# haowenz/chromap

Measured on AMD Instinct MI355X. Metric: M paired reads mapped/s (ATAC preset, GRCh38 index), higher is better.
Workload: dtype u64

## Files before the change

chromap_amd/csrc/cm_api.hip:

```cpp
#include <hip/hip_runtime.h>
#include <math.h>
#include <stdio.h>
#include <stdlib.h>
#include <string.h>

#include <string>
#include <vector>

#include "../../include/chromap_amd.h"
#include "cm_barcode_translate.h"
#include "cm_ctx.h"
#include "cm_kernels.h"
#include "cm_classes.h"
#include "cm_summary.h"
#include "cm_coop.h"
#include <chrono>
#include <mutex>
#include "cm_mapq_tables.h"

static thread_local std::string g_last_error;

static bool cm_debug_pool() { static const bool on = getenv("CM_DEBUG_POOL") != nullptr; return on; }
static thread_local std::string t_last_error;
void cm_set_error(cmgpu_ctx *ctx, const std::string &msg) {
// ... 90 lines not shown
    c->opt.spec = value ? 1 : 0;
    if (value < 0) { c->cls_seen = 0; memset(c->cls_age, 0, sizeof(c->cls_age)); }
  } else if (n == "debug_candidate_capacity") {
    if (value > 0 && cm_ensure_candidate_arrays(c, (uint64_t)value)) { cm_set_error(c, "out of device memory (candidates)"); return CMGPU_ENOMEM; }
    c->pred_m_ok = value > 0; c->m_cap = (uint64_t)value; c->pred_n = 0xffffffffu;
  } else if (n == "coop_profile") {
    if (value) { if (c->coop_prof.ensure(64 * 8)) return CMGPU_ENOMEM; CM_HIPCHECK(c, hipMemset(c->coop_prof.p, 0, 64 * 8)); } else c->coop_prof.release();
  } else if (n == "coop_run_table") {
    c->opt.coop_rb = (int)value;
  } else if (n == "coop") {
    c->opt.coop = (int)value;
  } else if (n == "pack_once") {
    c->opt.pack_once = value ? 1 : 0;
  } else if (n == "s3b_short") {
    c->opt.s3b_short = value ? 1 : 0;
  } else if (n == "s6_planes") {
    c->opt.s6_planes = value ? 1 : 0;
  } else if (n == "generic_kernels") {
    c->opt.generic_kernels = value ? 1 : 0;
  } else if (n == "item_limit") {
    c->opt.item_limit = value > 0 ? (uint64_t)value : 0xfffffff0ull;
  } else {
    cm_set_error(c, "unknown option " + n);
    return CMGPU_EINVAL;
  }
  return CMGPU_OK;
}

extern "C" int cmgpu_get_option(const cmgpu_ctx *c, const char *name, int64_t *value) {
  if (!c || !name || !value) return CMGPU_EINVAL;
  const std::string n(name);
  if (n == "probe_lookups_per_lane") *value = c->opt.probe_variant & 15;
  else if (n == "probe_pair_prefetch") *value = (c->opt.probe_variant & 16) ? 1 : 0;
  else if (n == "mm_chunks") *value = c->opt.mm_chunks;
  else if (n == "h2d_copy_blocks") *value = c->opt.h2d_kernel;
  else if (n == "d2h_copy_blocks") *value = c->opt.d2h_kernel;
  else if (n == "prep_kernel") *value = c->opt.prep_kernel;
  else if (n == "prep_tile_reads") *value = c->opt.prep_tile_reads;
  else if (n == "item_limit") *value = (int64_t)c->opt.item_limit;
  else if (n == "lanes") *value = c->opt.lanes;
  else if (n == "coop") *value = c->opt.coop;
  else if (n == "generic_kernels") *value = c->opt.generic_kernels;
  else if (n == "s3b_short") *value = c->opt.s3b_short;
  else if (n == "pack_once") *value = c->opt.pack_once;
  else if (n == "s6_planes") *value = c->opt.s6_planes;
  else if (n == "alloc_us") *value = (int64_t)(c->alloc_seconds * 1e6);
  else if (n == "alloc_draw_us") *value = (int64_t)(c->alloc_draw_seconds * 1e6);
  else if (n.rfind("coop_profile_", 0) == 0) {
    const int k = atoi(n.c_str() + 13);
    unsigned long long v = 0;
    if (k < 0 || k > 63 || !c->coop_prof.p || hipMemcpy(&v, (const unsigned long long *)c->coop_prof.p + k, 8, hipMemcpyDeviceToHost) != hipSuccess) return CMGPU_EINVAL;
    *value = (int64_t)v;
  }
  else if (n == "probe_table_buckets") *value = c->fmask ? (int64_t)c->fmask + 1 : (int64_t)c->bmask + 1;
  else return CMGPU_EINVAL;
  return CMGPU_OK;
}

extern "C" const char *cmgpu_last_error(const cmgpu_ctx *ctx) { return ctx ? ctx->err.c_str() : g_last_error.c_str(); }
// ... 658 lines not shown
  }
  return CMGPU_OK;
}
struct MmChunks {
  uint32_t n_chunks;
  uint32_t lo[CM_MM_CHUNKS + 1];
  uint64_t entries[CM_MM_CHUNKS];
  uint32_t part_off[CM_MM_CHUNKS + 1];
};
static uint32_t mm_chunk_count(const RangeRun &r) { return r.n >= (1u << 20) ? (uint32_t)r.c->opt.mm_chunks : (r.n >= (1u << 17) ? 2 : 1); }
static void mm_probe_grids(const cmgpu_ctx *c, MmChunks &k) {
  k.part_off[0] = 0;
  for (uint32_t ch = 0; ch < k.n_chunks; ++ch) k.part_off[ch + 1] = k.part_off[ch] + cm_probe_range_blocks(k.entries[ch], c->opt.probe_variant);
}
template <class Fill>
static int mm_fill_and_probe(RangeRun &r, const MmChunks &k, uint32_t mm_cap, Fill fill) {
  cmgpu_ctx *c = r.c;
  const unsigned long long *marks = (const unsigned long long *)c->mm_marks.p;
  CM_HIPCHECK(c, hipMemsetAsync(r.d.stats + CM_ST_PROBE_STEPS, 0, 2 * 8, r.s));
  for (uint32_t ch = 0; ch < k.n_chunks; ++ch) {
    fill(ch);
    CM_HIPCHECK(c, hipEventRecord(c->chunk_ev[ch], r.s));
    CM_HIPCHECK(c, hipStreamWaitEvent(c->stream2, c->chunk_ev[ch], 0));
    cm_launch_k_probe_range(r.d, marks + ch, k.entries[ch], mm_cap, (uint2 *)c->partials.p + k.part_off[ch], c->stream2, c->opt.probe_variant);
  }
  CM_HIPCHECK(c, hipEventRecord(c->chunk_ev[CM_MM_CHUNKS], c->stream2));
  CM_HIPCHECK(c, hipStreamWaitEvent(r.s, c->chunk_ev[CM_MM_CHUNKS], 0));
  cm_launch_k_probe_reduce(c->partials.p, k.part_off[k.n_chunks], r.d.stats + CM_ST_PROBE_STEPS, r.s);
  return CMGPU_OK;
}
static bool range_wants_planes(const cmgpu_ctx *c) { return c->ref_pl_words != 0 && c->opt.planes; }
static size_t read_planes_bytes(const cmgpu_ctx *c, uint32_t n2) { return (size_t)n2 * cm_read_pl_stride((c->max_read_len + 31) / 32) * 4 + 16; }
static int stage_minimizers_fused(RangeRun &r, bool flat) {
  cmgpu_ctx *c = r.c; CmDev &d = r.d; hipStream_t s = r.s;
  const uint32_t n = r.n, n2 = r.n2;
  int rc;
  const bool pl = !flat && c->opt.pack_once && cm_prep_mm_planes_supported(d, c->max_read_len);
  if (pl && range_wants_planes(c) && !c->read_planes.ensure(read_planes_bytes(c, n2))) {
    d.read_pl = (uint32_t *)c->read_planes.p; d.read_pl_w = (c->max_read_len + 31) / 32;
// ... 18 lines not shown
      chunk_pairs = pairs > chunk_pairs ? pairs : chunk_pairs;
      const uint64_t me = 2ull * pairs * (attempt == 0 ? (uint64_t)(c->max_read_len / 4 + 3) : per_read_bound);
      k.entries[ch] = me > cap ? cap : me;
    }
    mm_probe_grids(c, k);
    if (c->mm_hash.ensure((size_t)cap * 8 + 8) || c->mm_ps.ensure((size_t)cap * 4 + 4) || c->pr_val.ensure((size_t)cap * 8 + 8) ||
        (!flat && c->mm_stage.ensure(cm_prep_mm_stage_bytes(d, c->max_read_len, chunk_pairs) + 8)) ||
        c->pr_kind.ensure((size_t)cap + 4) || c->mm_cursor.ensure(8) || c->mm_marks.ensure((CM_MM_CHUNKS + 1) * 8) ||
        c->partials.ensure(((size_t)k.part_off[k.n_chunks] + 1) * 8 + cm_stats_partial_words(n) * 8)) {
      cm_set_error(c, "out of device memory (minimizers)"); return CMGPU_ENOMEM;
    }
    r.bind();
    CM_HIPCHECK(c, hipMemsetAsync(c->mm_cursor.p, 0, 8, s));
    CM_HIPCHECK(c, hipMemsetAsync(c->mm_marks.p, 0, 8, s));
    unsigned long long *cursor = (unsigned long long *)c->mm_cursor.p, *marks = (unsigned long long *)c->mm_marks.p;
    rc = mm_fill_and_probe(r, k, (uint32_t)cap, [&](uint32_t ch) {
      if (flat) cm_launch_k_prep_flat(d, k.lo[ch], k.lo[ch + 1], c->max_read_len, (uint32_t)c->opt.prep_tile_reads, (uint32_t)cap, cursor, s);
      else cm_launch_k_prep_mm(d, k.lo[ch], k.lo[ch + 1], c->max_read_len, (uint32_t)cap, cursor, s, c->mm_stage.p, pl);
      cm_launch_k_copy_u64(cursor, marks + ch + 1, s);
    });
    if (rc) return rc;
    d.mm_cap = (uint32_t)cap;
    CM_HIPCHECK(c, hipMemsetAsync(c->hv_cnt.p, 0, 256, s));
    cm_launch_k_s3a_count(d, n2, s);
    d.mm_cap = 0;
    if ((rc = scan_with_total(c, d.hit_tot, d.hit_off, n2, &r.hits_total, false))) return rc;
    CM_HIPCHECK(c, hipMemcpyAsync(r.n_heavy, c->hv_cnt.p, sizeof(r.n_heavy), hipMemcpyDeviceToHost, s));
    r.s3a_done = true;
    unsigned long long hm[CM_MM_CHUNKS + 1];
    CM_HIPCHECK(c, hipMemcpyAsync(hm, marks, ((size_t)k.n_chunks + 1) * 8, hipMemcpyDeviceToHost, s));
    CM_HIPCHECK(c, cm_stream_sync(s));
    const unsigned long long tot = hm[k.n_chunks];
    bool grid_short = false;
    if (attempt == 0 && tot <= cap)
      for (uint32_t ch = 0; ch < k.n_chunks; ++ch) grid_short = grid_short || hm[ch + 1] - hm[ch] > k.entries[ch];
    if (tot <= cap && !grid_short) { r.n_mm = (uint32_t)tot; break; }
    if (attempt == 1) { cm_set_error(c, "minimizer arrays overflowed twice"); return CMGPU_ECAPACITY; }
    cap = bound;
  }
  mark(c, "s0_s1_s2_trim_minimizers_probe");
// ... 38 lines not shown
    (void)hipDeviceGetStreamPriorityRange(&prio_least, &prio_greatest);
    CM_HIPCHECK(c, hipStreamCreateWithPriority(&c->stream_pack, hipStreamNonBlocking, prio_greatest));
  }
  CM_HIPCHECK(c, hipEventRecord(c->chunk_ev[1], r.s));
  CM_HIPCHECK(c, hipStreamWaitEvent(c->stream_pack, c->chunk_ev[1], 0));
  r.d.read_pl = (uint32_t *)c->read_planes.p; r.d.read_pl_w = (c->max_read_len + 31) / 32;
  cm_launch_k_pack_reads(r.d, r.n2, c->stream_pack);
  CM_HIPCHECK(c, hipEventRecord(c->chunk_ev[0], c->stream_pack));
  return CMGPU_OK;
}
static int stage_s3_candidates(RangeRun &r) {
  cmgpu_ctx *c = r.c; CmDev &d = r.d; hipStream_t s = r.s;
  const uint32_t n2 = r.n2;
  if (!r.s3a_done) {
    CM_HIPCHECK(c, hipMemsetAsync(c->hv_cnt.p, 0, 256, s));
    cm_launch_k_s3a_count(d, n2, s);
    CM_HIPCHECK(c, hipMemcpyAsync(r.n_heavy, c->hv_cnt.p, sizeof(r.n_heavy), hipMemcpyDeviceToHost, s));
    const int rc = scan_with_total(c, d.hit_tot, d.hit_off, n2, &r.hits_total);
    if (rc) return rc;
  }
  if (r.hits_total > r.limit) return CM_RC_SPLIT;
  r.n_hits = (uint32_t)r.hits_total;
  if (c->hbuf.ensure((size_t)r.n_hits * 8 + 8) || c->hcnt.ensure((size_t)r.n_hits + 4)) { cm_set_error(c, "out of device memory (hits)"); return CMGPU_ENOMEM; }
  r.bind();
  mark(c, "s3a_count");
  cm_launch_k_s3b_candidates(d, n2, c->max_read_len, s);
  const uint32_t *nh = r.n_heavy;
  cm_launch_k_s3b_heavy(d, nh, s, (c->opt.coop & 1) != 0, c->max_read_len);
  c->use_perm = (uint64_t)nh[CM_L_HIT_B256B] + nh[CM_L_HIT_SLAB] + nh[CM_L_HIT_B512] + nh[CM_L_HIT_B1024] > n2 / 65536 || (uint64_t)nh[CM_L_HIT_WAVE] + nh[CM_L_HIT_WAVE_SMALL] + nh[CM_L_HIT_B256A] > n2 / 256;
  if (c->opt.heavy_last) c->use_perm = c->opt.heavy_last > 0;
  if (c->use_perm) {
// ... 472 lines not shown
    if (c->last_range_lo != 0 || c->last_range_hi != c->n_pairs) { cm_set_error(c, "the batch was mapped in sub-batches"); return CMGPU_EINVAL; }
    if (capacity < n || !c->read_planes.p || c->read_planes.cap < n * 4) { cm_set_error(c, "debug array: buffer too small or array not resident"); return CMGPU_ECAPACITY; }
    CM_HIPCHECK(c, hipMemcpy(out, c->read_planes.p, n * 4, hipMemcpyDeviceToHost));
    return CMGPU_OK;
  }
  if (nm == "read_plain") {
    const uint64_t n = 2ull * c->n_pairs;
    if (n_out) *n_out = n;
    if (c->last_range_lo != 0 || c->last_range_hi != c->n_pairs) { cm_set_error(c, "the batch was mapped in sub-batches"); return CMGPU_EINVAL; }
    if (capacity < n || !c->read_plain.p || c->read_plain.cap < n) { cm_set_error(c, "debug array: buffer too small or array not resident"); return CMGPU_ECAPACITY; }
    std::vector<uint8_t> b(n);
    if (n) CM_HIPCHECK(c, hipMemcpy(b.data(), c->read_plain.p, n, hipMemcpyDeviceToHost));
    for (uint64_t i = 0; i < n; ++i) out[i] = b[i];
    return CMGPU_OK;
  }
  struct { const char *n; DevBuf *b; int per_pair; } tab[] = {
    {"rlen", &c->rlen, 0}, {"mm_cnt", &c->mm_cnt, 0}, {"hit_tot", &c->hit_tot, 0}, {"ncp", &c->ncp, 0}, {"ncn", &c->ncn, 0},
    {"resc_p", &c->resc_p, 0}, {"resc_n", &c->resc_n, 0}, {"mcp", &c->mcp, 0}, {"mcn", &c->mcn, 0}, {"fcp", &c->fcp, 0},
    {"fcn", &c->fcn, 0}, {"ndp", &c->ndp, 0}, {"ndn", &c->ndn, 0}, {"nv", &c->nv, 0}, {"pe_nbest", &c->pe_nbest, 1}};
  for (auto &t : tab)
    if (nm == t.n) {
      const uint64_t n = t.per_pair ? c->n_pairs : 2ull * c->n_pairs;
      if (n_out) *n_out = n;
      if (capacity < n || !t.b->p || t.b->cap < n * 4) { cm_set_error(c, "debug array: buffer too small or array not resident"); return CMGPU_ECAPACITY; }
      CM_HIPCHECK(c, hipMemcpy(out, t.b->p, n * 4, hipMemcpyDeviceToHost));
      return CMGPU_OK;
    }
  cm_set_error(c, "debug array: unknown name " + nm);
  return CMGPU_EINVAL;
}

extern "C" int cmgpu_debug_mapq(cmgpu_ctx *c, int kind, int32_t error_threshold, uint64_t n, const int32_t *reads, const int32_t *pairs,
// ... 603 lines not shown
```

chromap_amd/csrc/cm_ctx.h:

```cpp
#ifndef CM_CTX_H_
#define CM_CTX_H_
#include <hip/hip_runtime.h>

#include <string>
#include <thread>
#include <vector>

#include "../../include/chromap_amd.h"
#include "../../include/chromap_amd_debug.h"
#include "cm_types.h"

#define CM_MAX_EVENTS 32
#define CM_MAX_W_HOST 32
#define CM_BZ_SRC_NONE 0
#define CM_BZ_SRC_STORE 1
#define CM_BZ_SRC_UPLOAD 2
#define CM_BZ_SRC_DEVICE 3

struct DevBuf {
  void *p = nullptr;
  size_t cap = 0;
  bool owned = true;
  int ensure(size_t bytes);
  void release();
// ... 92 lines not shown
  int probe_variant = 1;
  int mm_chunks = CM_MM_CHUNKS;
  int prep_tile_reads = 32;
  int prep_kernel = 0;
  uint64_t item_limit = 0xfffffff0ull;
  int exchange_overlap = 0;
  int s3b_cap = 0;
  int lanes = 1;
  int heavy_mid = 0;
  int heavy_max[3] = {0, 0, 0};
  int heavy_last = 0;
  int spec = 1;
  int pack_once = 1;
  int s6_planes = 1;
  int s3b_short = 1;
  int generic_kernels = 0;
  int coop_rb = 0;
  int coop = 0xff;
};

struct cmgpu_ctx {
  CmOptions opt;
  int device = 0;
  hipStream_t stream = nullptr;
  hipStream_t stream2 = nullptr;
  hipStream_t stream_pack = nullptr;
  hipEvent_t chunk_ev[CM_MM_CHUNKS + 1] = {};
  std::string err;
  cmgpu_params hp;
  CmParams p;
// ... 191 lines not shown
```

chromap_amd/csrc/cm_kernels.h:

```cpp
#ifndef CM_KERNELS_H_
#define CM_KERNELS_H_
#include <hip/hip_runtime.h>

#include "cm_types.h"

#define CM_SLAB_CAP 65535u
#define CM_SLAB_BLOCKS 128u
#define CM_DECL_LAUNCH(kname) void cm_launch_##kname(const CmDev &d, uint32_t n, hipStream_t s);
void cm_launch_k_prep_count(const CmDev &d, uint32_t n_pairs, uint32_t max_read_len, hipStream_t s);
void cm_launch_k_mm_fill(const CmDev &d, uint32_t pair_lo, uint32_t pair_hi, uint32_t max_read_len, hipStream_t s);
void cm_launch_k_mm_marks(const uint32_t *mm_off, const uint32_t *lo, uint32_t n_marks, unsigned long long *marks, hipStream_t s);
bool cm_prep_mm_supported(const CmDev &d, uint32_t max_read_len);
bool cm_prep_flat_supported(const CmDev &d, uint32_t max_read_len, uint32_t tile_reads);
void cm_launch_k_prep_flat(const CmDev &d, uint32_t pair_lo, uint32_t pair_hi, uint32_t max_read_len, uint32_t tile_reads, uint32_t mm_cap,
                           unsigned long long *cursor, hipStream_t s);
uint32_t cm_prep_mm_pairs_per_block(const CmDev &d, uint32_t max_read_len);
size_t cm_prep_mm_stage_bytes(const CmDev &d, uint32_t max_read_len, uint32_t pairs);
bool cm_prep_mm_planes_supported(const CmDev &d, uint32_t max_read_len);
void cm_launch_k_prep_mm(const CmDev &d, uint32_t pair_lo, uint32_t pair_hi, uint32_t max_read_len, uint32_t mm_cap,
                         unsigned long long *cursor, hipStream_t s, void *gstage, bool planes = false);
uint32_t cm_probe_range_blocks(uint64_t max_entries, int variant);
void cm_launch_k_probe_range(const CmDev &d, const unsigned long long *range, uint64_t max_entries, uint32_t cap, void *partials, hipStream_t s, int variant);
void cm_launch_k_probe_reduce(const void *partials, uint32_t blocks, unsigned long long *counters, hipStream_t s);
CM_DECL_LAUNCH(k_s3a_count)
void cm_launch_k_sort_lists(const CmDev &d, int mode, hipStream_t s);
uint32_t cm_s3b_lane_cap(uint32_t max_read_len);
void cm_s3b_heavy_classes(uint32_t *hv_max, uint32_t *hv_big);
void cm_granted_classes(CmDev &d);
void cm_launch_k_s3b_heavy(const CmDev &d, const uint32_t *n_cls, hipStream_t s, bool coop, uint32_t max_read_len);
void cm_launch_k_s3b_candidates(const CmDev &d, uint32_t n, uint32_t max_read_len, hipStream_t s);
void cm_launch_k_s4a_rescue_count(const CmDev &d, uint32_t n, hipStream_t s, bool coop);
void cm_launch_k_s4b_rescue_merge(const CmDev &d, uint32_t n, hipStream_t s, bool coop, uint32_t max_read_len);
uint32_t cm_rescue_seg_cap(uint32_t n_reads);
void cm_launch_k_s4a_rescue_list(const CmDev &d, uint32_t n_reads, hipStream_t s, bool coop);
void cm_launch_k_s4b_rescue_list(const CmDev &d, uint32_t n_reads, hipStream_t s, bool coop, uint32_t max_read_len);
void cm_launch_k_s4c_reduce(const CmDev &d, uint32_t n, hipStream_t s, uint32_t coop);
void cm_launch_k_s5a_prepare(const CmDev &d, uint32_t n, hipStream_t s, bool coop);
void cm_launch_k_s5c_finalize(const CmDev &d, uint32_t n, hipStream_t s, bool coop);
void cm_launch_k_s5b_verify(const CmDev &d, uint32_t max_items, uint32_t n_reads, hipStream_t s);
// ... 29 lines not shown
```

chromap_amd/csrc/cm_kernels.hip:

```cpp
#include <hip/hip_runtime.h>
#include <stdio.h>
#include <string.h>
#include <cstring>
#include <atomic>
#include <map>
#include <mutex>
#include <type_traits>
#include <utility>
#include <rocprim/rocprim.hpp>

#include "cm_kernels.h"
#include "cm_stages.h"
#include "cm_classes.h"
#include "cm_coop.h"

#define CM_BLOCK 256

#define CM_ITEM_KERNEL(kname, fn, perm)                                      \
  __global__ __launch_bounds__(CM_BLOCK) void kname(CmDev d, uint32_t n) {   \
    if (d.abort && *d.abort) return;                                         \
    const uint32_t i = blockIdx.x * CM_BLOCK + threadIdx.x;                  \
    if (i < n) fn(d, d.perm ? d.perm[i] : i);                                \
  }

// ... 307 lines not shown
      d.mm_cnt[r] = (uint32_t)pref[b] - (uint32_t)pref[a];
      d.mm_off[r] = (uint32_t)(base + pref[a]);
    }
    __syncthreads();
  }
  if (valid && ri[t].fb) {
    const uint8_t *seq = cm_read_ptr(d, r);
    const uint32_t c = cm_minimizers_window<7>(seq, len, k, nullptr, nullptr, 0);
    const unsigned long long off = c ? atomicAdd(cursor, (unsigned long long)c) : 0ull;
    d.mm_cnt[r] = c;
    d.mm_off[r] = (uint32_t)off;
    if (c && off + c <= mm_cap) cm_minimizers_window<7>(seq, len, k, d.mm_hash + off, d.mm_ps + off, c);
  }
}

__global__ __launch_bounds__(CM_BLOCK) void k_s3a_count(CmDev d, uint32_t n) {
  const uint32_t i = blockIdx.x * CM_BLOCK + threadIdx.x;
  uint32_t tot = 0;
  if (i < n) {
    cm_s3a_count(d, i);
    tot = d.hit_tot[i];
  }
  const uint32_t cls = cm_hit_class(d, tot);
  __shared__ uint32_t sh_cnt[8], sh_base[8];
  if (threadIdx.x < 8) sh_cnt[threadIdx.x] = 0;
  __syncthreads();
  const uint32_t lane = threadIdx.x & 63u;
  const uint32_t ids[8] = {CM_L_HIT_WAVE, CM_L_HIT_B256A, CM_L_HIT_B256B, CM_L_HIT_SLAB, CM_L_HIT_G16, CM_L_HIT_B512, CM_L_HIT_WAVE_SMALL, CM_L_HIT_B1024};
  uint32_t slot = 0, mine = 8;
#pragma unroll
  for (uint32_t q = 0; q < 8; ++q) {
    const unsigned long long m = __ballot(cls == ids[q]);
// ... 1217 lines not shown
  }
}
void cm_launch_k_sum_u32(const uint32_t *in, uint32_t n, unsigned long long *out, hipStream_t s) {
  if (!n) return;
  uint32_t blocks = (n + CM_BLOCK * 8 - 1) / (CM_BLOCK * 8);
  if (blocks > 2048) blocks = 2048;
  hipLaunchKernelGGL(k_sum_u32, dim3(blocks), dim3(CM_BLOCK), 0, s, in, n, out);
}

static inline dim3 grid_for(uint32_t n) { return dim3((n + CM_BLOCK - 1) / CM_BLOCK); }

#define CM_LAUNCH(kname)                                                               \
  void cm_launch_##kname(const CmDev &d, uint32_t n, hipStream_t s) {                  \
    if (n) hipLaunchKernelGGL(kname, grid_for(n), dim3(CM_BLOCK), 0, s, d, n);         \
  }
void cm_launch_k_s3a_count(const CmDev &d, uint32_t n, hipStream_t s) {
  if (n) hipLaunchKernelGGL(k_s3a_count, grid_for(n), dim3(CM_BLOCK), 0, s, d, n);
}
uint32_t cm_s3b_lane_cap(uint32_t max_read_len) {
  uint32_t cap = max_read_len / 3;
  return cap < 16 ? 16 : (cap > 64 ? 64 : cap);
}
static inline bool cm_cls_on(const CmDev &d, uint32_t list) { return (d.cls_mask >> list) & 1ull; }
template <class K>
static bool cm_lds_optin(K kernel, size_t bytes) {
  if (bytes <= 64 * 1024) return true;
  if (bytes > 160 * 1024) return false;
  static std::mutex mu;
  static std::map<std::pair<int, const void *>, std::pair<size_t, size_t>> seen;
  int dev = 0;
  (void)hipGetDevice(&dev);
  std::lock_guard<std::mutex> lk(mu);
// ... 437 lines not shown
```

chromap_amd/csrc/cm_stages.h:

```cpp
#ifndef CM_STAGES_H_
#define CM_STAGES_H_

#include "cm_types.h"

struct CmModeAny {
  static constexpr bool kPe = false;
  static CM_HD bool split(const CmDev &d) { return d.p.split != 0; }
  static CM_HD bool single(const CmDev &d) { return d.p.single != 0; }
};
struct CmModePe {
  static constexpr bool kPe = true;
  static CM_HD bool split(const CmDev &) { return false; }
  static CM_HD bool single(const CmDev &) { return false; }
};

CM_HD uint32_t cm_c2u(uint8_t c) {
  const uint32_t u = c & 0xDFu;
  const uint32_t x = (u >> 1) & 3u;
  const uint32_t o = u - 0x41u;
  const bool acgt = o < 20u && ((0x80045u >> (o & 31u)) & 1u);
  return acgt ? x ^ (x >> 1) : 4u;
}
CM_HD uint8_t cm_negchar(uint8_t c) {
  const uint32_t v = 3u ^ cm_c2u(c);
// ... 411 lines not shown
  *s0_out = fa ? sa : sb;
  return true;
}

CM_HD uint32_t cm_brev32(uint32_t v);
CM_HD uint64_t cm_brev64(uint64_t v) { return ((uint64_t)cm_brev32((uint32_t)v) << 32) | cm_brev32((uint32_t)(v >> 32)); }
CM_HD uint64_t cm_mask64(uint32_t n) { return n >= 64u ? ~0ull : ((1ull << n) - 1ull); }
CM_HD void cm_trim_planes64(uint64_t a0, uint64_t a1, uint32_t l1, uint64_t b0, uint64_t b1, uint32_t l2, int min_overlap, int seed,
                            bool *found, uint32_t *s0_out) {
  const uint32_t down = 64u - l2;
  uint64_t B0 = ~(cm_brev64(b0) >> down), B1 = ~(cm_brev64(b1) >> down);
  const uint64_t seedmask = cm_mask64((uint32_t)seed);
  bool fa = false, fb = false;
  uint32_t sa = 0, sb = 0;
  const uint32_t last = l2 - (uint32_t)min_overlap;
  for (uint32_t s0 = 0; s0 <= last && !fa; ++s0) {
    const uint32_t n = l1 < l2 - s0 ? l1 : l2 - s0;
    const uint64_t D = ((a0 ^ B0) | (a1 ^ B1)) & cm_mask64(n);
    const bool ok = __builtin_popcountll(D) <= 1;
    if (ok && (D & seedmask) == 0) { fa = true; sa = s0; }
    if (ok && ((D >> seed) & seedmask) == 0 && !fb) { fb = true; sb = s0; }
    B0 >>= 1; B1 >>= 1;
  }
  *found = fa || fb;
  *s0_out = fa ? sa : sb;
}
struct CmPairPlanes { uint64_t p0[2], p1[2]; bool upper[2]; };

CM_HD void cm_s0_prep_ptr(const CmDev &d, uint32_t pair, const uint8_t *s1p, const uint8_t *s2p, const CmPairPlanes *pp = nullptr) {
  const uint32_t raw1 = d.ro0[pair + 1] - d.ro0[pair], raw2 = d.ro1[pair + 1] - d.ro1[pair];
  uint32_t len1 = raw1, len2 = raw2;
  bool ok = raw1 >= (uint32_t)d.p.min_read_len && (d.p.single || raw2 >= (uint32_t)d.p.min_read_len);
  if (d.bcb && !d.bc_ok[pair] && !d.p.bc_keep) ok = false;
  if (ok && d.p.trim && !d.p.single) {
    const uint8_t *s1 = s1p, *s2 = s2p;
    const bool swap = !(raw1 <= raw2);
    const uint8_t *rd1 = swap ? s2 : s1;
    const uint8_t *lng = swap ? s1 : s2;
    const uint32_t l1 = swap ? raw2 : raw1, l2 = swap ? raw1 : raw2;
    const int min_overlap = d.p.min_read_len;
    const int seed = min_overlap / 2;
    bool merged = false;
    bool fast = false, ffound = false;
    uint32_t fs0 = 0;
    if (seed >= 1 && seed <= 32 && 2 * seed <= min_overlap && l1 >= (uint32_t)min_overlap) {
      if (pp && l2 <= 64) {
        const int ia = swap ? 1 : 0, ib = swap ? 0 : 1;
        fast = pp->upper[0] && pp->upper[1];
        if (fast) cm_trim_planes64(pp->p0[ia], pp->p1[ia], l1, pp->p0[ib], pp->p1[ib], l2, min_overlap, seed, &ffound, &fs0);
      } else if (l2 <= 64) fast = cm_trim_fast<2>(rd1, l1, lng, l2, min_overlap, seed, &ffound, &fs0);
      else if (l2 <= 160) fast = cm_trim_fast<5>(rd1, l1, lng, l2, min_overlap, seed, &ffound, &fs0);
      else if (l2 <= 256) fast = cm_trim_fast<8>(rd1, l1, lng, l2, min_overlap, seed, &ffound, &fs0);
    }
    if (fast) {
      merged = true;
      if (ffound) {
        int overlap = (int)(l2 - fs0);
        int off2 = 0;
        if (overlap > (int)l1) { off2 = overlap - (int)l1; overlap = (int)l1; }
        const int t1 = swap ? overlap + off2 : overlap;
// ... 115 lines not shown
    if (ctl(pos, c < 4 ? 2 : 0)) { flush = false; break; }
  }
  if (flush && min_h != ~0ull) CM_EMIT(min_h, min_p);
#undef CM_EMIT
  return n;
}

template <int W, class Emit>
CM_HD uint32_t cm_minimizers_window_e(const uint8_t *seq, uint32_t len, int k, Emit &&emit) {
  return cm_minimizers_core<W>(seq, 0, len, true, k, W, [&](uint32_t n, uint64_t h, uint32_t p) { emit(n, h, p); return true; });
}

struct CmSrcBytes {
  const uint8_t *seq;
  CM_HD uint32_t operator()(uint32_t i) const { return cm_c2u(seq[i]); }
};
struct CmSrcPlanes {
  uint64_t p0, p1;
  CM_HD uint32_t operator()(uint32_t i) const { return ((uint32_t)(p0 >> i) & 1u) | (((uint32_t)(p1 >> i) & 1u) << 1); }
};
template <class Src, class Emit>
CM_HD uint32_t cm_minimizers_w7_oddk_seq_src(const Src &src, uint32_t len, int k, Emit &&emit) {
  const uint64_t shift = 2 * (uint64_t)(k - 1);
  const uint64_t mask = (((uint64_t)1) << (2 * k)) - 1;
  uint64_t fw = 0, rv = 0;
  uint64_t H[7];
#pragma unroll
  for (int j = 0; j < 7; ++j) H[j] = ~0ull;
  uint32_t sb = 0, fl = 0, bad = 0, n = 0;
  for (uint32_t pos = 0; pos < len; ++pos) {
    uint32_t c = src(pos);
    bad |= c >> 2;
    c &= 3;
    fw = ((fw << 2) | c) & mask;
// ... 32 lines not shown
  if (m_k < 7) {
    uint64_t v = ~0ull;
    int at = -1;
#pragma unroll
    for (int j = 0; j < 7; ++j)
      if (j >= 7 - (int)m_k && H[j] <= v) { v = H[j]; at = j; }
    if (at >= 0) { emit(n, v, ((len - 1 - (uint32_t)(6 - at)) << 1) | ((sb >> at) & 1u)); ++n; }
    return n;
  }
#pragma unroll
  for (int j = 0; j < 7; ++j)
    if ((fl >> j) & 1u) { emit(n, H[j], ((len - 1 - (uint32_t)(6 - j)) << 1) | ((sb >> j) & 1u)); ++n; }
  return n;
}

template <int HV, class Src, class Emit>
CM_HD uint32_t cm_minimizers_w7_oddk_blocks_src(const Src &src, uint32_t len, int k, Emit &&emit) {
  const uint64_t shift = 2 * (uint64_t)(k - 1);
  const uint64_t mask = (((uint64_t)1) << (2 * k)) - 1;
  uint64_t fw = 0, rv = 0;
  uint32_t bad = 0, n = 0;
  for (uint32_t pos = 0; pos + 1 < (uint32_t)k; ++pos) {
    uint32_t c = src(pos);
    bad |= c >> 2;
    c &= 3;
    fw = ((fw << 2) | c) & mask;
    rv = (rv >> 2) | (((uint64_t)(3 ^ c)) << shift);
  }
  const uint32_t m = len - (uint32_t)k + 1, nblk = (m + 6) / 7;
  uint64_t ep[7], Sp[7], SM[7];
  uint32_t sbp = 0;
#pragma unroll
  for (int j = 0; j < 7; ++j) { ep[j] = 0; Sp[j] = 0; SM[j] = 0; }
  for (uint32_t b = 0; b <= nblk; ++b) {
    uint64_t e[7];
    uint32_t sb = 0;
#pragma unroll
    for (int j = 0; j < 7; ++j) {
      const uint32_t i = 7 * b + (uint32_t)j;
      e[j] = 0;
      if (i < m) {
        uint32_t c = src(i + (uint32_t)k - 1);
        bad |= c >> 2;
        c &= 3;
        fw = ((fw << 2) | c) & mask;
        rv = (rv >> 2) | (((uint64_t)(3 ^ c)) << shift);
        const uint64_t h0 = cm_hash64_v<HV>(fw, mask), h1 = cm_hash64_v<HV>(rv, mask);
        const uint32_t strand = h0 < h1 ? 0u : 1u;
        e[j] = cm_hash64_v<HV>(strand ? h1 : h0, mask);
        sb |= strand << j;
      }
    }
    if (b == 0) {
      uint64_t v = e[0];
#pragma unroll
      for (int j = 1; j < 6; ++j) v = e[j] < v ? e[j] : v;
      if (e[6] == v) {
#pragma unroll
        for (int j = 0; j < 6; ++j) e[j] = e[j] == v ? ~0ull : e[j];
      }
    }
    uint64_t Mw[7];
    {
      uint64_t P = e[0];
      Mw[0] = Sp[0];
#pragma unroll
      for (int j = 1; j < 7; ++j) {
        Mw[j] = Sp[j] < P ? Sp[j] : P;
        P = e[j] < P ? e[j] : P;
      }
    }
    if (b > 0) {
      uint64_t PM = Mw[0];
#pragma unroll
      for (int j = 0; j < 7; ++j) {
        if (j > 0) PM = Mw[j] > PM ? Mw[j] : PM;
        const uint64_t F = j < 6 ? (SM[j < 6 ? j + 1 : 6] > PM ? SM[j < 6 ? j + 1 : 6] : PM) : PM;
        const uint32_t i = 7 * (b - 1) + (uint32_t)j;
        if (F == ep[j] && i < m) { emit(n, ep[j], ((i + (uint32_t)k - 1) << 1) | ((sbp >> j) & 1u)); ++n; }
      }
    }
    SM[6] = Mw[6];
    Sp[6] = e[6];
#pragma unroll
    for (int j = 5; j >= 0; --j) {
      SM[j] = Mw[j] > SM[j + 1] ? Mw[j] : SM[j + 1];
      Sp[j] = e[j] < Sp[j + 1] ? e[j] : Sp[j + 1];
    }
#pragma unroll
    for (int j = 0; j < 7; ++j) ep[j] = e[j];
    sbp = sb;
  }
  if (bad) return ~0u;
  return n;
}
template <class Src, class Emit>
CM_HD uint32_t cm_minimizers_w7_oddk_src(const Src &src, uint32_t len, int k, Emit &&emit) {
  if (len < (uint32_t)k + 6) return cm_minimizers_w7_oddk_seq_src(src, len, k, emit);
  if (2 * k == 34) return cm_minimizers_w7_oddk_blocks_src<0>(src, len, k, emit);
  if (2 * k > 32 && 2 * k <= 52) return cm_minimizers_w7_oddk_blocks_src<1>(src, len, k, emit);
  return cm_minimizers_w7_oddk_blocks_src<2>(src, len, k, emit);
}
template <class Emit>
CM_HD uint32_t cm_minimizers_w7_oddk_seq(const uint8_t *seq, uint32_t len, int k, Emit &&emit) {
  return cm_minimizers_w7_oddk_seq_src(CmSrcBytes{seq}, len, k, emit);
}
template <int HV, class Emit>
CM_HD uint32_t cm_minimizers_w7_oddk_blocks(const uint8_t *seq, uint32_t len, int k, Emit &&emit) {
  return cm_minimizers_w7_oddk_blocks_src<HV>(CmSrcBytes{seq}, len, k, emit);
}
template <class Emit>
CM_HD uint32_t cm_minimizers_w7_oddk(const uint8_t *seq, uint32_t len, int k, Emit &&emit) {
  return cm_minimizers_w7_oddk_src(CmSrcBytes{seq}, len, k, emit);
}

CM_HD uint32_t cm_mmf_pack4(uint32_t w, uint32_t *bad4) {
  const uint32_t x = (w >> 1) & 0x03030303u;
  const uint32_t code = x ^ ((x >> 1) & 0x01010101u);
  const uint32_t b0 = code & 0x01010101u, b1 = (code >> 1) & 0x01010101u;
  const uint32_t canon = 0x41414141u + 2u * b0 + 6u * b1 + 11u * (b0 & b1);
  const uint32_t diff = (w & 0xDFDFDFDFu) ^ canon;
  const uint32_t nz = ((diff & 0x7F7F7F7Fu) + 0x7F7F7F7Fu) | diff;
  const uint32_t m = (nz >> 7) & 0x01010101u;
  *bad4 = (m | (m >> 7) | (m >> 14) | (m >> 21)) & 0xFu;
// ... 2688 lines not shown
```

Baseline: 633.5.

## Overlap s3a counting with probe chunks and speed up minimizer and overlap inner loops

Runs the s3a hit-count kernel per minimizer chunk on the secondary stream, so it overlaps the remaining prep and probe work instead of running after all chunks finish. It also rewrites the k=17 windowed-minimizer block loop to bias hash keys into double-float form and use v_min_f64/v_max_f64 for 64-bit min/max, with a cursor-based code source. It also skips the popcount in the pair-overlap scan unless a seed check passes and updates the mask incrementally. Adds debug array exports for round2 and hit lists. The float-key trick depends on hashes fitting in 52 bits and on f64 ordering matching integer ordering for those keys.

```diff
diff --git a/chromap_amd/csrc/cm_api.hip b/chromap_amd/csrc/cm_api.hip
--- a/chromap_amd/csrc/cm_api.hip
+++ b/chromap_amd/csrc/cm_api.hip
@@ -128,6 +128,8 @@
     c->opt.pack_once = value ? 1 : 0;
   } else if (n == "s3b_short") {
     c->opt.s3b_short = value ? 1 : 0;
+  } else if (n == "s3a_chunked") {
+    c->opt.s3a_chunked = value ? 1 : 0;
   } else if (n == "s6_planes") {
     c->opt.s6_planes = value ? 1 : 0;
   } else if (n == "generic_kernels") {
@@ -157,6 +159,7 @@
   else if (n == "generic_kernels") *value = c->opt.generic_kernels;
   else if (n == "s3b_short") *value = c->opt.s3b_short;
   else if (n == "pack_once") *value = c->opt.pack_once;
+  else if (n == "s3a_chunked") *value = c->opt.s3a_chunked;
   else if (n == "s6_planes") *value = c->opt.s6_planes;
   else if (n == "alloc_us") *value = (int64_t)(c->alloc_seconds * 1e6);
   else if (n == "alloc_draw_us") *value = (int64_t)(c->alloc_draw_seconds * 1e6);
@@ -845,7 +848,7 @@
   for (uint32_t ch = 0; ch < k.n_chunks; ++ch) k.part_off[ch + 1] = k.part_off[ch] + cm_probe_range_blocks(k.entries[ch], c->opt.probe_variant);
 }
 template <class Fill>
-static int mm_fill_and_probe(RangeRun &r, const MmChunks &k, uint32_t mm_cap, Fill fill) {
+static int mm_fill_and_probe(RangeRun &r, const MmChunks &k, uint32_t mm_cap, Fill fill, const CmDev *s3a = nullptr) {
   cmgpu_ctx *c = r.c;
   const unsigned long long *marks = (const unsigned long long *)c->mm_marks.p;
   CM_HIPCHECK(c, hipMemsetAsync(r.d.stats + CM_ST_PROBE_STEPS, 0, 2 * 8, r.s));
@@ -854,6 +857,7 @@
     CM_HIPCHECK(c, hipEventRecord(c->chunk_ev[ch], r.s));
     CM_HIPCHECK(c, hipStreamWaitEvent(c->stream2, c->chunk_ev[ch], 0));
     cm_launch_k_probe_range(r.d, marks + ch, k.entries[ch], mm_cap, (uint2 *)c->partials.p + k.part_off[ch], c->stream2, c->opt.probe_variant);
+    if (s3a) cm_launch_k_s3a_count(*s3a, 2 * k.lo[ch], 2 * k.lo[ch + 1], c->stream2);
   }
   CM_HIPCHECK(c, hipEventRecord(c->chunk_ev[CM_MM_CHUNKS], c->stream2));
   CM_HIPCHECK(c, hipStreamWaitEvent(r.s, c->chunk_ev[CM_MM_CHUNKS], 0));
@@ -902,16 +906,17 @@
     CM_HIPCHECK(c, hipMemsetAsync(c->mm_cursor.p, 0, 8, s));
     CM_HIPCHECK(c, hipMemsetAsync(c->mm_marks.p, 0, 8, s));
     unsigned long long *cursor = (unsigned long long *)c->mm_cursor.p, *marks = (unsigned long long *)c->mm_marks.p;
+    CM_HIPCHECK(c, hipMemsetAsync(c->hv_cnt.p, 0, 256, s));
+    CmDev d3 = d;
+    d3.mm_cap = (uint32_t)cap;
+    const bool chunked = c->opt.s3a_chunked != 0;
     rc = mm_fill_and_probe(r, k, (uint32_t)cap, [&](uint32_t ch) {
       if (flat) cm_launch_k_prep_flat(d, k.lo[ch], k.lo[ch + 1], c->max_read_len, (uint32_t)c->opt.prep_tile_reads, (uint32_t)cap, cursor, s);
       else cm_launch_k_prep_mm(d, k.lo[ch], k.lo[ch + 1], c->max_read_len, (uint32_t)cap, cursor, s, c->mm_stage.p, pl);
       cm_launch_k_copy_u64(cursor, marks + ch + 1, s);
-    });
+    }, chunked ? &d3 : nullptr);
     if (rc) return rc;
-    d.mm_cap = (uint32_t)cap;
-    CM_HIPCHECK(c, hipMemsetAsync(c->hv_cnt.p, 0, 256, s));
-    cm_launch_k_s3a_count(d, n2, s);
-    d.mm_cap = 0;
+    if (!chunked) cm_launch_k_s3a_count(d3, 0, n2, s);
     if ((rc = scan_with_total(c, d.hit_tot, d.hit_off, n2, &r.hits_total, false))) return rc;
     CM_HIPCHECK(c, hipMemcpyAsync(r.n_heavy, c->hv_cnt.p, sizeof(r.n_heavy), hipMemcpyDeviceToHost, s));
     r.s3a_done = true;
@@ -980,7 +985,7 @@
   const uint32_t n2 = r.n2;
   if (!r.s3a_done) {
     CM_HIPCHECK(c, hipMemsetAsync(c->hv_cnt.p, 0, 256, s));
-    cm_launch_k_s3a_count(d, n2, s);
+    cm_launch_k_s3a_count(d, 0, n2, s);
     CM_HIPCHECK(c, hipMemcpyAsync(r.n_heavy, c->hv_cnt.p, sizeof(r.n_heavy), hipMemcpyDeviceToHost, s));
     const int rc = scan_with_total(c, d.hit_tot, d.hit_off, n2, &r.hits_total);
     if (rc) return rc;
@@ -1483,8 +1488,36 @@
     for (uint64_t i = 0; i < n; ++i) out[i] = b[i];
     return CMGPU_OK;
   }
+  if (nm == "round2") {
+    const uint64_t n = 2ull * c->n_pairs;
+    if (n_out) *n_out = n;
+    if (capacity < n || !c->round2.p || c->round2.cap < n) { cm_set_error(c, "debug array: buffer too small or array not resident"); return CMGPU_ECAPACITY; }
+    std::vector<uint8_t> b(n);
+    if (n) CM_HIPCHECK(c, hipMemcpy(b.data(), c->round2.p, n, hipMemcpyDeviceToHost));
+    for (uint64_t i = 0; i < n; ++i) out[i] = b[i];
+    return CMGPU_OK;
+  }
+  if (nm == "hit_lists") {
+    static const uint32_t ids[8] = {CM_L_HIT_WAVE, CM_L_HIT_B256A, CM_L_HIT_B256B, CM_L_HIT_SLAB, CM_L_HIT_G16, CM_L_HIT_B512, CM_L_HIT_WAVE_SMALL, CM_L_HIT_B1024};
+    if (c->last_range_lo != 0 || c->last_range_hi != c->n_pairs) { cm_set_error(c, "the batch was mapped in sub-batches"); return CMGPU_EINVAL; }
+    const size_t stride = 2 * (size_t)c->n_pairs + 1;
+    uint32_t cnt[64];
+    if (!c->hv_cnt.p || c->hv_cnt.cap < 256 || !c->hv_list.p) { cm_set_error(c, "debug array: array not resident"); return CMGPU_ECAPACITY; }
+    CM_HIPCHECK(c, hipMemcpy(cnt, c->hv_cnt.p, 256, hipMemcpyDeviceToHost));
+    uint64_t n = 0;
+    for (uint32_t id : ids) n += cnt[id];
+    if (n_out) *n_out = n;
+    if (capacity < n) { cm_set_error(c, "debug array: buffer too small"); return CMGPU_ECAPACITY; }
+    uint64_t at = 0;
+    for (uint32_t id : ids) {
+      if (cnt[id] > stride || c->hv_list.cap < ((size_t)id * stride + cnt[id]) * 4) { cm_set_error(c, "debug array: list longer than its room"); return CMGPU_ECAPACITY; }
+      if (cnt[id]) CM_HIPCHECK(c, hipMemcpy(out + at, (const uint32_t *)c->hv_list.p + (size_t)id * stride, (size_t)cnt[id] * 4, hipMemcpyDeviceToHost));
+      at += cnt[id];
+    }
+    return CMGPU_OK;
+  }
   struct { const char *n; DevBuf *b; int per_pair; } tab[] = {
-    {"rlen", &c->rlen, 0}, {"mm_cnt", &c->mm_cnt, 0}, {"hit_tot", &c->hit_tot, 0}, {"ncp", &c->ncp, 0}, {"ncn", &c->ncn, 0},
+    {"rlen", &c->rlen, 0}, {"rep_len", &c->rep_len, 0}, {"rep_cnt", &c->rep_cnt, 0}, {"mm_cnt", &c->mm_cnt, 0}, {"hit_tot", &c->hit_tot, 0}, {"ncp", &c->ncp, 0}, {"ncn", &c->ncn, 0},
     {"resc_p", &c->resc_p, 0}, {"resc_n", &c->resc_n, 0}, {"mcp", &c->mcp, 0}, {"mcn", &c->mcn, 0}, {"fcp", &c->fcp, 0},
     {"fcn", &c->fcn, 0}, {"ndp", &c->ndp, 0}, {"ndn", &c->ndn, 0}, {"nv", &c->nv, 0}, {"pe_nbest", &c->pe_nbest, 1}};
   for (auto &t : tab)
diff --git a/chromap_amd/csrc/cm_ctx.h b/chromap_amd/csrc/cm_ctx.h
--- a/chromap_amd/csrc/cm_ctx.h
+++ b/chromap_amd/csrc/cm_ctx.h
@@ -130,6 +130,7 @@
   int pack_once = 1;
   int s6_planes = 1;
   int s3b_short = 1;
+  int s3a_chunked = 1;
   int generic_kernels = 0;
   int coop_rb = 0;
   int coop = 0xff;
diff --git a/chromap_amd/csrc/cm_kernels.h b/chromap_amd/csrc/cm_kernels.h
--- a/chromap_amd/csrc/cm_kernels.h
+++ b/chromap_amd/csrc/cm_kernels.h
@@ -22,7 +22,7 @@
 uint32_t cm_probe_range_blocks(uint64_t max_entries, int variant);
 void cm_launch_k_probe_range(const CmDev &d, const unsigned long long *range, uint64_t max_entries, uint32_t cap, void *partials, hipStream_t s, int variant);
 void cm_launch_k_probe_reduce(const void *partials, uint32_t blocks, unsigned long long *counters, hipStream_t s);
-CM_DECL_LAUNCH(k_s3a_count)
+void cm_launch_k_s3a_count(const CmDev &d, uint32_t first, uint32_t n, hipStream_t s);
 void cm_launch_k_sort_lists(const CmDev &d, int mode, hipStream_t s);
 uint32_t cm_s3b_lane_cap(uint32_t max_read_len);
 void cm_s3b_heavy_classes(uint32_t *hv_max, uint32_t *hv_big);
diff --git a/chromap_amd/csrc/cm_kernels.hip b/chromap_amd/csrc/cm_kernels.hip
--- a/chromap_amd/csrc/cm_kernels.hip
+++ b/chromap_amd/csrc/cm_kernels.hip
@@ -345,8 +345,8 @@
   }
 }
 
-__global__ __launch_bounds__(CM_BLOCK) void k_s3a_count(CmDev d, uint32_t n) {
-  const uint32_t i = blockIdx.x * CM_BLOCK + threadIdx.x;
+__global__ __launch_bounds__(CM_BLOCK) void k_s3a_count(CmDev d, uint32_t first, uint32_t n) {
+  const uint32_t i = first + blockIdx.x * CM_BLOCK + threadIdx.x;
   uint32_t tot = 0;
   if (i < n) {
     cm_s3a_count(d, i);
@@ -1594,8 +1594,8 @@
   void cm_launch_##kname(const CmDev &d, uint32_t n, hipStream_t s) {                  \
     if (n) hipLaunchKernelGGL(kname, grid_for(n), dim3(CM_BLOCK), 0, s, d, n);         \
   }
-void cm_launch_k_s3a_count(const CmDev &d, uint32_t n, hipStream_t s) {
-  if (n) hipLaunchKernelGGL(k_s3a_count, grid_for(n), dim3(CM_BLOCK), 0, s, d, n);
+void cm_launch_k_s3a_count(const CmDev &d, uint32_t first, uint32_t n, hipStream_t s) {
+  if (n > first) hipLaunchKernelGGL(k_s3a_count, grid_for(n - first), dim3(CM_BLOCK), 0, s, d, first, n);
 }
 uint32_t cm_s3b_lane_cap(uint32_t max_read_len) {
   uint32_t cap = max_read_len / 3;
diff --git a/chromap_amd/csrc/cm_stages.h b/chromap_amd/csrc/cm_stages.h
--- a/chromap_amd/csrc/cm_stages.h
+++ b/chromap_amd/csrc/cm_stages.h
@@ -449,20 +449,25 @@
   bool fa = false, fb = false;
   uint32_t sa = 0, sb = 0;
   const uint32_t last = l2 - (uint32_t)min_overlap;
+  uint64_t mk = cm_mask64(l1);
   for (uint32_t s0 = 0; s0 <= last && !fa; ++s0) {
-    const uint32_t n = l1 < l2 - s0 ? l1 : l2 - s0;
-    const uint64_t D = ((a0 ^ B0) | (a1 ^ B1)) & cm_mask64(n);
-    const bool ok = __builtin_popcountll(D) <= 1;
-    if (ok && (D & seedmask) == 0) { fa = true; sa = s0; }
-    if (ok && ((D >> seed) & seedmask) == 0 && !fb) { fb = true; sb = s0; }
+    const uint64_t D = ((a0 ^ B0) | (a1 ^ B1)) & mk;
+    const bool ca = (D & seedmask) == 0, cb = ((D >> seed) & seedmask) == 0 && !fb;
+    if (ca || cb) {
+      const bool ok = __builtin_popcountll(D) <= 1;
+      if (ok && ca) { fa = true; sa = s0; }
+      if (ok && cb) { fb = true; sb = s0; }
+    }
     B0 >>= 1; B1 >>= 1;
+    if (l2 - s0 <= l1) mk >>= 1;
   }
   *found = fa || fb;
   *s0_out = fa ? sa : sb;
 }
 struct CmPairPlanes { uint64_t p0[2], p1[2]; bool upper[2]; };
 
-CM_HD void cm_s0_prep_ptr(const CmDev &d, uint32_t pair, const uint8_t *s1p, const uint8_t *s2p, const CmPairPlanes *pp = nullptr) {
+CM_HD void cm_s0_prep_ptr(const CmDev &d, uint32_t pair, const uint8_t *s1p, const uint8_t *s2p, const CmPairPlanes *pp = nullptr,
+                          bool allow_fast = true) {
   const uint32_t raw1 = d.ro0[pair + 1] - d.ro0[pair], raw2 = d.ro1[pair + 1] - d.ro1[pair];
   uint32_t len1 = raw1, len2 = raw2;
   bool ok = raw1 >= (uint32_t)d.p.min_read_len && (d.p.single || raw2 >= (uint32_t)d.p.min_read_len);
@@ -478,7 +483,7 @@
     bool merged = false;
     bool fast = false, ffound = false;
     uint32_t fs0 = 0;
-    if (seed >= 1 && seed <= 32 && 2 * seed <= min_overlap && l1 >= (uint32_t)min_overlap) {
+    if (allow_fast && seed >= 1 && seed <= 32 && 2 * seed <= min_overlap && l1 >= (uint32_t)min_overlap) {
       if (pp && l2 <= 64) {
         const int ia = swap ? 1 : 0, ib = swap ? 0 : 1;
         fast = pp->upper[0] && pp->upper[1];
@@ -624,10 +629,22 @@
 struct CmSrcBytes {
   const uint8_t *seq;
   CM_HD uint32_t operator()(uint32_t i) const { return cm_c2u(seq[i]); }
+  struct Cur {
+    const uint8_t *at;
+    CM_HD uint32_t operator()(int j) const { return cm_c2u(at[j]); }
+    CM_HD void next() { at += 7; }
+  };
+  CM_HD Cur cur(uint32_t i) const { return Cur{seq + i}; }
 };
 struct CmSrcPlanes {
   uint64_t p0, p1;
   CM_HD uint32_t operator()(uint32_t i) const { return ((uint32_t)(p0 >> i) & 1u) | (((uint32_t)(p1 >> i) & 1u) << 1); }
+  struct Cur {
+    uint64_t q0, q1;
+    CM_HD uint32_t operator()(int j) const { return (((uint32_t)q0 >> j) & 1u) | ((((uint32_t)q1 >> j) & 1u) << 1); }
+    CM_HD void next() { q0 >>= 7; q1 >>= 7; }
+  };
+  CM_HD Cur cur(uint32_t i) const { return Cur{p0 >> i, p1 >> i}; }
 };
 template <class Src, class Emit>
 CM_HD uint32_t cm_minimizers_w7_oddk_seq_src(const Src &src, uint32_t len, int k, Emit &&emit) {
@@ -690,8 +707,51 @@
   return n;
 }
 
-template <int HV, class Src, class Emit>
+#define CM_KEY_BIAS 0x4330000000000000ull
+#define CM_KEY_STRUCK 0x4340000000000000ull
+#define CM_KEY_HASH 0x000FFFFFFFFFFFFFull
+CM_HD uint64_t cm_key_min_int(uint64_t a, uint64_t b) { return b < a ? b : a; }
+CM_HD uint64_t cm_key_max_int(uint64_t a, uint64_t b) { return b > a ? b : a; }
+CM_HD uint64_t cm_key_min_f64(uint64_t a, uint64_t b) {
+#if defined(__HIP_DEVICE_COMPILE__)
+  uint64_t r;
+  asm("v_min_f64 %0, %1, %2" : "=v"(r) : "v"(a), "v"(b));
+  return r;
+#else
+  double x, y;
+  __builtin_memcpy(&x, &a, 8);
+  __builtin_memcpy(&y, &b, 8);
+  return y < x ? b : a;
+#endif
+}
+CM_HD uint64_t cm_key_max_f64(uint64_t a, uint64_t b) {
+#if defined(__HIP_DEVICE_COMPILE__)
+  uint64_t r;
+  asm("v_max_f64 %0, %1, %2" : "=v"(r) : "v"(a), "v"(b));
+  return r;
+#else
+  double x, y;
+  __builtin_memcpy(&x, &a, 8);
+  __builtin_memcpy(&y, &b, 8);
+  return y > x ? b : a;
+#endif
+}
+#if defined(__HIP_DEVICE_COMPILE__)
+#define CM_ORD_KEYS 2
+#else
+#define CM_ORD_KEYS 1
+#endif
+template <int ORD>
+struct CmOrd {
+  static constexpr uint64_t kPad = ORD ? CM_KEY_BIAS : 0ull, kStruck = ORD ? CM_KEY_STRUCK : ~0ull;
+  static CM_HD uint64_t key(uint64_t h) { return ORD ? h | CM_KEY_BIAS : h; }
+  static CM_HD uint64_t hash(uint64_t x) { return ORD ? x & CM_KEY_HASH : x; }
+  static CM_HD uint64_t mn(uint64_t a, uint64_t b) { return ORD == 2 ? cm_key_min_f64(a, b) : cm_key_min_int(a, b); }
+  static CM_HD uint64_t mx(uint64_t a, uint64_t b) { return ORD == 2 ? cm_key_max_f64(a, b) : cm_key_max_int(a, b); }
+};
+template <int HV, int ORD, class Src, class Emit>
 CM_HD uint32_t cm_minimizers_w7_oddk_blocks_src(const Src &src, uint32_t len, int k, Emit &&emit) {
+  using O = CmOrd<ORD>;
   const uint64_t shift = 2 * (uint64_t)(k - 1);
   const uint64_t mask = (((uint64_t)1) << (2 * k)) - 1;
   uint64_t fw = 0, rv = 0;
@@ -706,34 +766,39 @@
   const uint32_t m = len - (uint32_t)k + 1, nblk = (m + 6) / 7;
   uint64_t ep[7], Sp[7], SM[7];
   uint32_t sbp = 0;
-#pragma unroll
-  for (int j = 0; j < 7; ++j) { ep[j] = 0; Sp[j] = 0; SM[j] = 0; }
-  for (uint32_t b = 0; b <= nblk; ++b) {
+  const uint32_t pp0 = (uint32_t)k - 8u;
+  uint32_t pp = pp0, sbk = 0;
+  int32_t rem = (int32_t)m;
+#pragma unroll
+  for (int j = 0; j < 7; ++j) { ep[j] = O::kPad; Sp[j] = O::kPad; SM[j] = O::kPad; }
+  auto codes = src.cur((uint32_t)k - 1);
+  for (uint32_t b = 0; ORD ? true : b <= nblk; ++b, rem -= 7, pp += 7) {
     uint64_t e[7];
     uint32_t sb = 0;
+    sbk <<= 7;
 #pragma unroll
     for (int j = 0; j < 7; ++j) {
       const uint32_t i = 7 * b + (uint32_t)j;
-      e[j] = 0;
-      if (i < m) {
-        uint32_t c = src(i + (uint32_t)k - 1);
+      e[j] = O::kPad;
+      if (ORD ? j < rem : i < m) {
+        uint32_t c = ORD ? codes(j) : src(i + (uint32_t)k - 1);
         bad |= c >> 2;
         c &= 3;
         fw = ((fw << 2) | c) & mask;
         rv = (rv >> 2) | (((uint64_t)(3 ^ c)) << shift);
         const uint64_t h0 = cm_hash64_v<HV>(fw, mask), h1 = cm_hash64_v<HV>(rv, mask);
         const uint32_t strand = h0 < h1 ? 0u : 1u;
-        e[j] = cm_hash64_v<HV>(strand ? h1 : h0, mask);
-        sb |= strand << j;
-      }
-    }
-    if (b == 0) {
+        e[j] = O::key(cm_hash64_v<HV>(strand ? h1 : h0, mask));
+        if (ORD) sbk |= strand << j; else sb |= strand << j;
+      }
+    }
+    if (ORD ? pp == pp0 : b == 0) {
       uint64_t v = e[0];
 #pragma unroll
-      for (int j = 1; j < 6; ++j) v = e[j] < v ? e[j] : v;
+      for (int j = 1; j < 6; ++j) v = O::mn(e[j], v);
       if (e[6] == v) {
 #pragma unroll
-        for (int j = 0; j < 6; ++j) e[j] = e[j] == v ? ~0ull : e[j];
+        for (int j = 0; j < 6; ++j) e[j] = e[j] == v ? O::kStruck : e[j];
       }
     }
     uint64_t Mw[7];
@@ -742,30 +807,34 @@
       Mw[0] = Sp[0];
 #pragma unroll
       for (int j = 1; j < 7; ++j) {
-        Mw[j] = Sp[j] < P ? Sp[j] : P;
-        P = e[j] < P ? e[j] : P;
-      }
-    }
-    if (b > 0) {
+        Mw[j] = O::mn(Sp[j], P);
+        P = O::mn(e[j], P);
+      }
+    }
+    if (ORD ? pp != pp0 : b > 0) {
       uint64_t PM = Mw[0];
 #pragma unroll
       for (int j = 0; j < 7; ++j) {
-        if (j > 0) PM = Mw[j] > PM ? Mw[j] : PM;
-        const uint64_t F = j < 6 ? (SM[j < 6 ? j + 1 : 6] > PM ? SM[j < 6 ? j + 1 : 6] : PM) : PM;
+        if (j > 0) PM = O::mx(Mw[j], PM);
+        const uint64_t F = j < 6 ? O::mx(SM[j < 6 ? j + 1 : 6], PM) : PM;
         const uint32_t i = 7 * (b - 1) + (uint32_t)j;
-        if (F == ep[j] && i < m) { emit(n, ep[j], ((i + (uint32_t)k - 1) << 1) | ((sbp >> j) & 1u)); ++n; }
+        if (ORD) {
+          if (F == ep[j] && j < rem + 7) { emit(n, O::hash(ep[j]), ((pp + (uint32_t)j) << 1) | ((sbk >> (7 + j)) & 1u)); ++n; }
+        } else if (F == ep[j] && i < m) { emit(n, ep[j], ((i + (uint32_t)k - 1) << 1) | ((sbp >> j) & 1u)); ++n; }
       }
     }
     SM[6] = Mw[6];
     Sp[6] = e[6];
 #pragma unroll
     for (int j = 5; j >= 0; --j) {
-      SM[j] = Mw[j] > SM[j + 1] ? Mw[j] : SM[j + 1];
-      Sp[j] = e[j] < Sp[j + 1] ? e[j] : Sp[j + 1];
+      SM[j] = O::mx(Mw[j], SM[j + 1]);
+      Sp[j] = O::mn(e[j], Sp[j + 1]);
     }
 #pragma unroll
     for (int j = 0; j < 7; ++j) ep[j] = e[j];
     sbp = sb;
+    if (ORD) codes.next();
+    if (ORD && rem <= 0) break;
   }
   if (bad) return ~0u;
   return n;
@@ -773,9 +842,9 @@
 template <class Src, class Emit>
 CM_HD uint32_t cm_minimizers_w7_oddk_src(const Src &src, uint32_t len, int k, Emit &&emit) {
   if (len < (uint32_t)k + 6) return cm_minimizers_w7_oddk_seq_src(src, len, k, emit);
-  if (2 * k == 34) return cm_minimizers_w7_oddk_blocks_src<0>(src, len, k, emit);
-  if (2 * k > 32 && 2 * k <= 52) return cm_minimizers_w7_oddk_blocks_src<1>(src, len, k, emit);
-  return cm_minimizers_w7_oddk_blocks_src<2>(src, len, k, emit);
+  if (2 * k == 34) return cm_minimizers_w7_oddk_blocks_src<0, CM_ORD_KEYS>(src, len, k, emit);
+  if (2 * k > 32 && 2 * k <= 52) return cm_minimizers_w7_oddk_blocks_src<1, 0>(src, len, k, emit);
+  return cm_minimizers_w7_oddk_blocks_src<2, 0>(src, len, k, emit);
 }
 template <class Emit>
 CM_HD uint32_t cm_minimizers_w7_oddk_seq(const uint8_t *seq, uint32_t len, int k, Emit &&emit) {
@@ -783,7 +852,7 @@
 }
 template <int HV, class Emit>
 CM_HD uint32_t cm_minimizers_w7_oddk_blocks(const uint8_t *seq, uint32_t len, int k, Emit &&emit) {
-  return cm_minimizers_w7_oddk_blocks_src<HV>(CmSrcBytes{seq}, len, k, emit);
+  return cm_minimizers_w7_oddk_blocks_src<HV, 0>(CmSrcBytes{seq}, len, k, emit);
 }
 template <class Emit>
 CM_HD uint32_t cm_minimizers_w7_oddk(const uint8_t *seq, uint32_t len, int k, Emit &&emit) {
```

Result: no change. 637.0 (median of 3 runs) (+0.5%).
